# David-Wobrock/image-processing-graph-laplacian

Hardware: AMD Instinct MI355X
Metric: filtered Mpixels/sec @ 4K img, 0.5% samples; PSNR vs PETSc ref (higher is better)
Workload: dtype f32 (f32 storage and accumulation; MFMA operands split into f16 hi+lo pairs = 22 significant bits)

## Files before the change

### image-processing-graph-laplacian_amd/csrc/band_plan.hpp

```cpp
#pragma once
#include <cstdint>
#include <vector>

#if defined(__HIP__) || defined(__CUDACC__)
#define GLF_BAND_HD __host__ __device__
#else
#define GLF_BAND_HD
#endif

namespace glf {

#ifndef BAND_MAXROWS_X
#define BAND_MAXROWS_X 128
#endif
constexpr int BAND_MAXROWS = BAND_MAXROWS_X;
constexpr int BAND_RMAX = 1023;
constexpr unsigned BAND_EMPTY = 0x0000FFFFu;
#ifndef BAND_PB_X
#define BAND_PB_X 2
#endif
#ifndef BAND_NW_X
#define BAND_NW_X 8
#endif
constexpr int BAND_PB = BAND_PB_X, BAND_NW = BAND_NW_X;
// ... 55 lines not shown
    const int i1 = BSEP_KSTEP * ks + BSEP_KSTEP - 1 < count - 1 ? BSEP_KSTEP * ks + BSEP_KSTEP - 1 : count - 1;
    const int first = gcol[band_sep_col(clo, BSEP_KSTEP * ks, nc)], last = gcol[band_sep_col(clo, i1, nc)];
    return first - p1 >= rad || p0 - last >= rad;
}
GLF_BAND_HD inline uint64_t band_sep_tile_entries(const int *gcol, int nc, int width, int tc0, int tile_px, int d, int rad, bool all)
{
    int clo, count;
    band_sep_tile_cols(gcol, nc, width, tc0, tile_px, d, &clo, &count);
    uint64_t n = 0;
    for (int ks = 0; ks < band_sep_ksteps(count); ++ks)
        for (int pt = 0; pt < tile_px / 32; ++pt)
            if (all || !band_sep_block_dead(gcol, nc, clo, count, ks, tc0 + 32 * pt, tc0 + 32 * pt + 31, rad)) n += (uint64_t)BSEP_KSTEP * 32u;
    return n;
}

struct BandGeom {
    int rad = 0;
    double D2 = 0.0;
    std::vector<int> rows, cols, dcmax;
    bool init(const int *grows, int nr, const int *gcols, int nc, double s_loc);
    unsigned band_of(int r) const;
    unsigned window(int cmin, int cmax, int dr, int shift) const;
};

}
```

### image-processing-graph-laplacian_amd/csrc/ctx.hip

```cpp
#include "glf_internal.hpp"

#include <cmath>
#include <cstdlib>

extern "C" {

const char *glf_strerror(int status)
{
    switch (status) {
    case GLF_OK: return "ok";
    case GLF_ERR_INVALID: return "invalid argument";
    case GLF_ERR_NOMEM: return "out of memory";
    case GLF_ERR_HIP: return "HIP runtime error";
    case GLF_ERR_NODEVICE: return "no usable gfx950 device";
    case GLF_ERR_COMM: return "collective callback failed";
    case GLF_ERR_NOCONV: return "eigensolver did not converge";
    case GLF_ERR_IO: return "image I/O error";
    case GLF_ERR_UNSUPPORTED: return "unsupported";
    default: return "unknown status";
    }
}

int glf_ctx_create(glf_ctx **out, int device, void *hip_stream)
{
// ... 33 lines not shown
        }
    for (auto &row : ctx->mv_ev)
        for (auto &e : row)
            if (hipEventCreate(&e) != hipSuccess) {
                delete ctx;
                return GLF_ERR_HIP;
            }
    ctx->comm.rank = 0;
    ctx->comm.size = 1;
    if (const char *mode = std::getenv("GLF_CONTRACTION")) {
        if (std::strcmp(mode, "f32") == 0) ctx->contraction = GLF_CONTRACT_F32_MFMA;
        else if (std::strcmp(mode, "f16s") == 0) ctx->contraction = GLF_CONTRACT_F16_SPLIT;
        else fprintf(stderr, "glf: ignoring GLF_CONTRACTION=%s (expected f32 or f16s)\n", mode);
    }
    if (const char *dbg = std::getenv("GLF_POOL_DEBUG")) ctx->pool_debug = dbg[0] && dbg[0] != '0';
    for (const char *key : {"NYS_PATH", "DEG_PATH", "MV_PATH", "ROWPASS", "ROWPASS_OP", "SWEEP_COLPASS", "COLPASS", "NYS_NO_LUT", "NO_ECR", "NO_NARROW", "NO_FUSED_FILTER", "FILTER_FORM", "BAND_NOSKIP", "PIX_BAND", "EIG_SHARD", "ZMFMA_GROUPS", "GS", "RESIDUAL", "OPERAND_MAXIMA", "VERBOSE"}) {
        char name[32];
        std::snprintf(name, sizeof(name), "GLF_%s", key);
        if (const char *v = std::getenv(name))
            if (glf_ctx_set_tuning(ctx, key, v) != GLF_OK) fprintf(stderr, "glf: ignoring %s=%s\n", name, v);
    }
    *out = ctx;
    return GLF_OK;
}

int glf_ctx_set_tuning(glf_ctx *ctx, const char *key, const char *value)
{
    if (!ctx || !key) return GLF_ERR_INVALID;
    const bool unset = !value || !value[0] || !std::strcmp(value, "auto") || !std::strcmp(value, "default");
    auto is = [&](const char *s) { return value && !std::strcmp(value, s); };
    auto flag = [&]() { return !unset && !is("0"); };
// ... 14 lines not shown
    } else if (!std::strcmp(key, "SWEEP_COLPASS")) {
        if (!unset && !is("segments") && !is("samples")) return GLF_ERR_INVALID;
        t.sweep_samples = is("samples");
    } else if (!std::strcmp(key, "COLPASS")) {
        if (!unset && !is("ws") && !is("v1")) return GLF_ERR_INVALID;
        t.colpass = is("v1") ? 1 : 0;
    } else if (!std::strcmp(key, "NYS_NO_LUT")) t.nys_no_lut = flag();
    else if (!std::strcmp(key, "NO_ECR")) t.no_ecr = flag();
    else if (!std::strcmp(key, "NO_NARROW")) t.no_narrow = flag();
    else if (!std::strcmp(key, "NO_FUSED_FILTER")) t.no_fused_filter = flag();
    else if (!std::strcmp(key, "FILTER_FORM")) {
        if (!unset && !is("sep") && !is("vec") && !is("phi")) return GLF_ERR_INVALID;
        t.filter_form = is("sep") ? 1 : is("vec") ? 2 : is("phi") ? 3 : 0;
    } else if (!std::strcmp(key, "BAND_NOSKIP")) t.band_noskip = flag();
    else if (!std::strcmp(key, "PIX_BAND")) t.pix_band = flag();
    else if (!std::strcmp(key, "ZMFMA_GROUPS")) t.zmfma_groups = flag();
    else if (!std::strcmp(key, "EIG_SHARD")) t.eig_shard = unset ? 0 : is("0") ? 2 : 1;
    else if (!std::strcmp(key, "GS")) {
        if (!unset && !is("seq") && !is("gram")) return GLF_ERR_INVALID;
        t.gs_seq = is("seq");
    } else if (!std::strcmp(key, "RESIDUAL")) {
        if (!unset && !is("sweep") && !is("derived")) return GLF_ERR_INVALID;
        t.residual_sweep = is("sweep");
    } else if (!std::strcmp(key, "OPERAND_MAXIMA")) {
        if (!unset && !is("sweep") && !is("carried")) return GLF_ERR_INVALID;
        t.operand_maxima_sweep = is("sweep");
    } else if (!std::strcmp(key, "VERBOSE")) t.verbose = flag();
    else return GLF_ERR_INVALID;
    return GLF_OK;
}

size_t glf_ctx_cached_bytes(const glf_ctx *ctx)
{
    size_t total = 0;
    if (ctx)
        for (const glf_pool_block &b : ctx->pool)
            if (!b.in_use) total += b.bytes;
    return total;
}

int glf_ctx_debug_violations(const glf_ctx *ctx)
{
    if (!ctx || !ctx->pool_debug) return -1;
    return ctx->pool_violations;
}

int glf_ctx_destroy(glf_ctx *ctx)
{
    if (!ctx) return GLF_OK;
    (void)hipSetDevice(ctx->device);
    (void)hipStreamSynchronize(ctx->stream);
    for (auto &e : ctx->ev)
        if (e) (void)hipEventDestroy(e);
    for (auto &row : ctx->mv_ev)
// ... 331 lines not shown
```

### image-processing-graph-laplacian_amd/csrc/glf_internal.hpp

```cpp
#pragma once

#include <hip/hip_runtime.h>

#include <cmath>
#include <cstdarg>
#include <cstdint>
#include <cstdio>
#include <cstring>
#include <limits>
#include <type_traits>
#include <utility>
#include <vector>

#include "../../include/glf.h"
#include "band_plan.hpp"

struct glf_pool_block {
    void *p;
    size_t bytes;
    bool in_use;
    unsigned last_call = 0;
};

struct glf_tuning {
// ... 2 lines not shown
    int mv_path = 0;
    int rowpass = 0;
    int rowpass_op = 0;
    bool sweep_samples = false;
    int colpass = 0;
    bool nys_no_lut = false;
    bool no_ecr = false;
    bool gs_seq = false;
    bool residual_sweep = false;
    bool zmfma_groups = false;
    int eig_shard = 0;
    bool no_fused_filter = false;
    int filter_form = 0;
    bool band_noskip = false;
    bool pix_band = false;
    bool no_narrow = false;
    bool operand_maxima_sweep = false;
    bool verbose = false;
};

struct glf_native_comm;

struct glf_ctx {
    std::vector<glf_pool_block> pool;
    int device = 0;
    hipStream_t stream = nullptr;
    bool owns_stream = false;
    glf_comm comm{};
    bool has_comm = false;
    glf_native_comm *native = nullptr;
// ... 9 lines not shown
    hipEvent_t cp_ev[2][CP_RING] = {};
    int mv_pending = 0;
    unsigned call_no = 0;
    int mv_count = 0;
    int narrow_sweeps = 0;
    double mv_ms = 0.0, mv_bytes = 0.0;
    float *x0_block = nullptr;
    unsigned x0_p = 0, x0_m = 0, x0_ld = 0;
    unsigned long long x0_seed = 0;
    float *x0_orth = nullptr;
    double *x0_orth_norms = nullptr;
    int x0_orth_form = 0;
    bool x0_orth_fused = false;
    int contraction = GLF_CONTRACT_F16_SPLIT;
    struct { int skipping = 0, lut = 0; } nys_note;
    struct { int path = 0, shape = 0, skipping = 0, chunks = 0, mgroups = 0; double entries = 0.0; } deg_note;
    struct { unsigned kernels = 0, ld = 0, panels = 0, proj_blocks = 0, apply_blocks = 0, strided = 0; } flt_note;
    void *pinned = nullptr;
    void *band_cache[2] = {nullptr, nullptr};
    bool rank_valid = false;
    float rank_s_val = 0.f;
    int rank_R = 0;
    void *rank_ftab = nullptr;
    void *rank_ff = nullptr;
    bool pool_debug = false;
    int pool_violations = 0;
    glf_tuning tune;
};

struct glf_graph {
// ... 660 lines not shown
```

### image-processing-graph-laplacian_amd/csrc/host_util.cpp

```cpp
#include <algorithm>
#include <cmath>
#include <cstdint>
#include <cstdlib>
#include <vector>

#include "../../include/glf.h"
#include "band_plan.hpp"
#include "phi_compact.hpp"
#include "robust_loss.hpp"

namespace {

inline uint64_t rotl64(uint64_t x, int k) { return (x << k) | (x >> (64 - k)); }

struct Xoshiro256ss {
    uint64_t s[4];
    explicit Xoshiro256ss(uint64_t seed)
    {
        for (int i = 0; i < 4; ++i) {
            uint64_t z = (seed += 0x9E3779B97F4A7C15ull);
            z = (z ^ (z >> 30)) * 0xBF58476D1CE4E5B9ull;
            z = (z ^ (z >> 27)) * 0x94D049BB133111EBull;
            s[i] = z ^ (z >> 31);
        }
// ... 201 lines not shown
                    unsigned h = glf::BAND_EMPTY;
                    for (int i = glf::BAND_PAIR * j; i < std::min(nb, glf::BAND_PAIR * (j + 1)); ++i) {
                        const int dr = std::abs(trow0 + w - geom.rows[alo + i]);
                        h = glf::band_win_hull(h, dr < geom.rad ? win[(size_t)dr * nt + t] : glf::BAND_EMPTY);
                    }
                    if (u) u[j] = h;
                    if (glf::band_win_live(h)) steps += (h >> 16) - (h & 0xFFFFu) + 1;
                }
            }
        }
    }
    if (ksteps) *ksteps = steps;
    return GLF_OK;
}

int glf_cluster_update(unsigned k, unsigned dim, const double *scale, const double *sums, const uint64_t *counts, const double *cent_prev,
                       double *cent)
{
    return cluster_update(k, dim, scale, sums, counts, cent_prev, cent);
}

int glf_cluster_update_w(unsigned k, unsigned dim, const double *scale, const double *sums, const double *mass, const double *cent_prev,
                         double *cent)
{
    return cluster_update(k, dim, scale, sums, mass, cent_prev, cent);
}

int glf_cluster_seed(const double *rows, size_t n, unsigned dim, unsigned k, uint64_t seed, double *cent)
{
    return cluster_seed(rows, nullptr, n, dim, k, seed, cent);
// ... 318 lines not shown
```

### image-processing-graph-laplacian_amd/csrc/nystroem_band.inc

```

#ifndef BAND_SETPRIO
#define BAND_SETPRIO 1
#endif
#ifndef BAND_PCOPY
#define BAND_PCOPY 16
#endif
#ifndef BAND_NBUF
#define BAND_NBUF 2
#endif
constexpr unsigned BAND_PSTRIDE = 4u * BAND_PCOPY;
#ifndef BAND_GROWS
#define BAND_GROWS 4
#endif
constexpr int BAND_G = BAND_GROWS;
__host__ __device__ constexpr inline int band_chunk_bytes(int mb) { return mb * 2048 + 256; }
constexpr int BAND_WB = 6;
__host__ __device__ constexpr inline int band_stage_chunks(bool samples)
{
    return samples && 2 * BAND_WB > BAND_NBUF * BAND_G ? 2 * BAND_WB : BAND_NBUF * BAND_G;
}
__host__ __device__ inline unsigned band_lds_bytes(int mb, int nw, int rad, int ksc, bool samples, bool plut = true)
{
    return (plut ? 256u * BAND_PSTRIDE : 0u) + (unsigned)band_stage_chunks(samples) * (unsigned)band_chunk_bytes(mb) + 4u * (unsigned)(rad + 1) + 64u * (unsigned)ksc + 4u * BAND_MAXROWS * (unsigned)(1 + 2 * nw) + 16u;
}
// ... 584 lines not shown
        }
        __syncthreads();
        if (tid < LD) {
            double tot = 0.0;
            for (int w = 0; w < NW; ++w) tot += (double)red[w * LD + tid];
            cpartial[((size_t)blockIdx.y * gridDim.x + blockIdx.x) * LD + tid] = tot;
        }
    }
}

struct BandTables {
    int rad = 0, nr = 0, nc = 0, ksc = 0, width = 0;
    int tile_px = 0, ntiles_px = 0, ntiles_s = 0;
    bool ok = false;
    DevBuf<unsigned> blob;
    size_t o_pexp = 0, o_grid = 0, o_rb_px = 0, o_win_px = 0, o_rb_s = 0, o_win_s = 0, o_dcmax = 0;
    const float *tab() const { return reinterpret_cast<const float *>(blob.p); }
    const float *pexp() const { return reinterpret_cast<const float *>(blob.p + o_pexp); }
    const int *grow() const { return reinterpret_cast<const int *>(blob.p + o_grid); }
    const int *gcol() const { return grow() + nr; }
    const unsigned *rowband_px() const { return blob.p + o_rb_px; }
    const unsigned *win_px() const { return blob.p + o_win_px; }
    const unsigned *rowband_s() const { return blob.p + o_rb_s; }
    const unsigned *win_s() const { return blob.p + o_win_s; }
    const int *dcmax() const { return reinterpret_cast<const int *>(blob.p + o_dcmax); }
    std::vector<unsigned> h_rowband_px;
    double er15_rowsum = 0.0;
    int dc0() const { return geom.dcmax.empty() ? -1 : geom.dcmax[0]; }
    int cols_near_tile(int t) const
    {
        int lo = 0, n = 0;
// ... 39 lines not shown
        nc = g.nc;
        ksc = (int)ceil_div(nc, 16);
        width = width_;
        tile_px = tile_px_;
        hrows = g.rows;
        if (nr > 65535 || ksc > 65535) return GLF_ERR_UNSUPPORTED;
        ntiles_px = want_px ? (int)ceil_div(width, tile_px) : 0;
        ntiles_s = want_s ? (int)ceil_div(nc, 32) : 0;
        const size_t n_tab = 256 + 2 * (size_t)(rad + 1);
        o_pexp = (n_tab + 3) / 4 * 4;
        o_grid = o_pexp + 256 * (size_t)BAND_PCOPY;
        o_rb_px = o_grid + (size_t)nr + nc;
        o_win_px = o_rb_px + (want_px ? (size_t)height : 0);
        o_rb_s = o_win_px + (size_t)rad * ntiles_px;
        o_win_s = o_rb_s + (want_s ? (size_t)nr : 0);
        o_dcmax = o_win_s + (size_t)rad * ntiles_s;
        std::vector<unsigned> h(o_dcmax + (size_t)rad);
        float *htab = reinterpret_cast<float *>(h.data());
        for (int e = 0; e < 256; ++e) htab[e] = (float)std::exp2(-(double)coef.s_val * e * e);
        for (int d = 0; d <= rad; ++d) {
            const double t = (double)coef.s_loc * (double)d * (double)d;
            htab[256 + d] = d < rad ? (float)std::exp2(-t) : 0.f;
            htab[256 + rad + 1 + d] = d < rad ? (float)std::exp2((double)NYS_F16_KSCALE_LOG2 - t) : 0.f;
        }
        for (int i = 0; i < 256 * BAND_PCOPY; ++i) reinterpret_cast<float *>(h.data())[o_pexp + i] = htab[i / BAND_PCOPY];
        for (int a = 0; a < nr; ++a) h[o_grid + a] = (unsigned)g.rows[a];
        for (int b = 0; b < nc; ++b) h[o_grid + nr + b] = (unsigned)g.cols[b];
        const std::vector<int> &dcmax = geom.dcmax;
        for (int dr = 0; dr < rad; ++dr) h[o_dcmax + dr] = (unsigned)dcmax[dr];
        int maxband = 0;
        if (want_px) {
// ... 16 lines not shown
            for (int dr = 0; dr < rad; ++dr) {
                if (dcmax[dr] < 0) continue;
                double n = 0.0;
                for (int b = 0; b < nc; ++b) n += (double)(std::min(width - 1, g.cols[b] + dcmax[dr]) - std::max(0, g.cols[b] - dcmax[dr]) + 1);
                pairs_dr[dr] = n;
            }
        }
        if (want_s) {
            for (int a = 0; a < nr; ++a) {
                const unsigned rb = band_of(g.rows[a]);
                h[o_rb_s + a] = rb;
                maxband = std::max(maxband, (int)(rb >> 16) - (int)(rb & 0xFFFF) + 1);
            }
            for (int dr = 0; dr < rad; ++dr)
                for (int t = 0; t < ntiles_s; ++t) h[o_win_s + (size_t)dr * ntiles_s + t] = geom.window(g.cols[t * 32], g.cols[std::min(nc, (t + 1) * 32) - 1], dr, BAND_BLOCK_SHIFT);
            pairs_dr_s.assign(rad, 0.0);
            for (int dr = 0; dr < rad; ++dr) {
                if (dcmax[dr] < 0) continue;
                double n = 0.0;
                int lo = 0, hi = 0;
                for (int b = 0; b < nc; ++b) {
                    while (lo < nc && g.cols[lo] < g.cols[b] - dcmax[dr]) ++lo;
                    while (hi < nc && g.cols[hi] <= g.cols[b] + dcmax[dr]) ++hi;
                    n += (double)(hi - lo);
                }
                pairs_dr_s[dr] = n;
            }
        }
        if (maxband + 8 > BAND_MAXROWS) return GLF_ERR_UNSUPPORTED;
        GLF_TRY(blob.alloc(ctx, h.size()));
// ... 28 lines not shown
    e->s_loc = coef.s_loc;
    e->s_val = coef.s_val;
    e->width = width;
    e->height = height;
    e->tile_px = tile_px;
    const int rc = e->bt.build(ctx, g, coef, width, height, tile_px, px, !px);
    if (rc != GLF_OK) {
        delete e;
        e = nullptr;
        return rc;
    }
    *out = &e->bt;
    return GLF_OK;
}

#ifndef BAND_NW_S_X
#define BAND_NW_S_X 8
#endif
constexpr int BAND_NW_S = BAND_NW_S_X;

template <int MB, int NS = 0, PixGen G = PixGen::Grey>
static int launch_band_px(glf_ctx *ctx, const BandTables &bt, const uint8_t *d_img, int row0, int nrows, const unsigned char *chunks,
                          const float *inv, float *phi, int phi_ld, const uint8_t *d_mask, const uint32_t *d_idx, unsigned p, int raster,
                          double *cpartial, unsigned long long *evaluated, const BandFilter *flt = nullptr, int64_t pix0 = 0, float nsval = 0.f)
{
    if constexpr (G != PixGen::Grey)
        if (flt || cpartial) return set_error(ctx, GLF_ERR_INVALID, "k_band: the colour and 16-bit formats have no filter epilogue");
    if constexpr (NS == 0 && G == PixGen::Grey)
        if (flt && flt->sig.nsig > 0) {
            if (flt->sig.nsig >= BANDV_MAXNC) return set_error(ctx, GLF_ERR_INVALID, "k_band: %d signal planes", flt->sig.nsig);
// ... 9 lines not shown
    hipLaunchKernelGGL(kern, grid, dim3(BAND_NW * 64), lds, ctx->stream, d_img, bt.width, row0, bt.grow(), bt.gcol(), bt.nr, bt.nc,
                       bt.ksc, bt.tab(), bt.pexp(), bt.rad, bt.rowband_px(), bt.win_px(), bt.ntiles_px, chunks, inv, phi, phi_ld, d_mask, d_idx, p, raster,
                       cpartial, (const float *)nullptr, 0, (const double *)nullptr, 0.f, evaluated, row0 + nrows, flt ? flt->w : (const float *)nullptr,
                       flt ? flt->gain : 0.f, flt ? flt->ysub : 0.f, flt ? flt->out : (uint8_t *)nullptr, flt ? flt->zf : (float *)nullptr,
                       flt ? flt->corr : (float *)nullptr, pix0, flt ? flt->sig : BandSignals{}, ctx->tune.band_noskip ? 1 : 0, nsval);
    GLF_LAUNCH_CHECK(ctx);
    return GLF_OK;
}
inline size_t band_px_wgs(const BandTables &bt, int nrows) { return (size_t)bt.ntiles_px * (size_t)ceil_div(nrows, BAND_NW); }

template <int MB, PixGen G = PixGen::Grey>
static int launch_band_samples(glf_ctx *ctx, const BandTables &bt, const uint8_t *svals, int a0, int nrows, const unsigned char *chunks,
                               const float *inv, float *Y, int y_ld, const float *X, int x_ld, const double *degree, float alpha,
                               unsigned long long *evaluated, float nsval = 0.f)
{
    auto kern = k_band<MB, 1, BAND_NW_S, true, 0, G>;
    const unsigned lds = band_lds_bytes(MB, BAND_NW_S, bt.rad, bt.ksc, true, G == PixGen::Grey);
    GLF_HIP(ctx, hipFuncSetAttribute(reinterpret_cast<const void *>(kern), hipFuncAttributeMaxDynamicSharedMemorySize, (int)lds));
    const dim3 grid((unsigned)bt.ntiles_s, (unsigned)ceil_div(nrows, BAND_NW_S));
    hipLaunchKernelGGL(kern, grid, dim3(BAND_NW_S * 64), lds, ctx->stream, svals, bt.nc, a0, bt.grow(), bt.gcol(), bt.nr, bt.nc, bt.ksc,
                       bt.tab(), bt.pexp(), bt.rad, bt.rowband_s(), bt.win_s(), bt.ntiles_s, chunks, inv, Y, y_ld, (const uint8_t *)nullptr,
                       (const uint32_t *)nullptr, 0u, 1, (double *)nullptr, X, x_ld, degree, alpha, evaluated, a0 + nrows, (const float *)nullptr, 0.f,
                       0.f, (uint8_t *)nullptr, (float *)nullptr, (float *)nullptr, (int64_t)0, BandSignals{}, 0, nsval);
    GLF_LAUNCH_CHECK(ctx);
    return GLF_OK;
}

static int band_prep(glf_ctx *ctx, const float *X, unsigned x_ld, const float *colscale, const void *svals, bool raw, int nr, int nc, int ksc, int mb,
                     unsigned char *chunks, int nch = 1)
{
// ... 120 lines not shown
```

### image-processing-graph-laplacian_amd/glf.py

```python
import collections
import ctypes as C
import functools
import os

import numpy as np
import torch

_HERE = os.path.dirname(os.path.abspath(__file__))
LIB_PATH = os.environ.get("GLF_LIBRARY", os.path.join(_HERE, "libglf.so"))
if not os.path.exists(LIB_PATH):
    raise ImportError(
        "libglf.so not found at %s: build it with `make` (or __graft_entry__.build()); "
        "there is no CPU fallback for the HIP path" % LIB_PATH)
_lib = C.CDLL(LIB_PATH)

OK = 0
ERR_INVALID, ERR_NOMEM, ERR_HIP, ERR_NODEVICE, ERR_COMM, ERR_NOCONV, ERR_IO, ERR_UNSUPPORTED = range(-1, -9, -1)
MAT_DENSE, MAT_DIAG, MAT_KERNEL_B = 0, 1, 2
ROWS_NA, ROWS_SAMPLE_FIRST, ROWS_RASTER = 0, 1, 2
KERNEL_BILATERAL, KERNEL_PHOTOMETRIC, KERNEL_SPATIAL, KERNEL_NLM, KERNEL_BILATERAL_RGB, KERNEL_BILATERAL_U16 = 0, 1, 2, 3, 4, 5
KERNEL_BILATERAL_F32 = 6
KERNEL_BILATERAL_RGBF32 = 7
CONTRACT_F32_MFMA, CONTRACT_F16_SPLIT = 1, 2
FILTER_REFERENCE, FILTER_POC, FILTER_SMOOTH, FILTER_SHARPEN = 0, 1, 2, 3
SAMPLING_UNIFORM, SAMPLING_RANDOM = 0, 1
MULTI_RCCL, MULTI_LOOPBACK = 0, 1
RCCL_ID_BYTES = 128

EXPORTS = [
    "glf_strerror", "glf_ctx_create", "glf_ctx_destroy", "glf_ctx_synchronize", "glf_ctx_last_error",
    "glf_ctx_device_info", "glf_ctx_set_tuning", "glf_ctx_set_comm", "glf_rccl_unique_id", "glf_ctx_set_comm_rccl", "glf_ctx_comm_info", "glf_ctx_comm_counters", "glf_multi_create", "glf_multi_destroy",
    "glf_multi_size", "glf_multi_ctx", "glf_multi_last_error", "glf_multi_image_processing", "glf_shard_rows", "glf_band_plan", "glf_ctx_set_contraction", "glf_malloc", "glf_free", "glf_memcpy_h2d", "glf_memcpy_d2h",
    "glf_memset", "glf_mat_create_dense", "glf_mat_create_diag", "glf_mat_destroy", "glf_mat_get_column", "glf_Sampling",
    "glf_host_free", "glf_random_vectors", "glf_synth_image", "glf_RandomSampling", "glf_ComputeAffinityMatrices",
    "glf_ComputeLaplacianMatrix", "glf_InversePowerIteration", "glf_OrthonormaliseVecs", "glf_NormaliseVecs",
    "glf_InverseDiagMat", "glf_Nystroem", "glf_Permutation", "glf_ComputeResultFromLaplacian", "glf_Sinkhorn", "glf_SinkhornRows", "glf_Orthogonalisation",
    "glf_options_default", "glf_image_processing", "glf_image_processing_capture", "glf_ctx_debug_violations", "glf_ctx_cached_bytes", "glf_image_processing_batch", "glf_EntireComputation", "glf_read_png", "glf_write_png", "glf_read_png_rgb", "glf_write_png_rgb",
    "glf_image_processing_signals", "glf_multi_image_processing_signals",
    "glf_image_processing_rgb", "glf_multi_image_processing_rgb", "glf_image_processing_rgb_capture",
    "glf_image_processing_u16", "glf_multi_image_processing_u16", "glf_image_processing_u16_capture", "glf_read_png16", "glf_write_png16",
    "glf_image_processing_rgb_signals", "glf_image_processing_u16_signals",
    "glf_multi_image_processing_rgb_signals", "glf_multi_image_processing_u16_signals",
    "glf_image_processing_f32", "glf_image_processing_f32_capture", "glf_image_processing_f32_signals",
    "glf_multi_image_processing_f32", "glf_multi_image_processing_f32_signals", "glf_read_pfm", "glf_write_pfm",
    "glf_image_processing_rgbf32", "glf_image_processing_rgbf32_capture", "glf_image_processing_rgbf32_signals",
    "glf_multi_image_processing_rgbf32", "glf_multi_image_processing_rgbf32_signals", "glf_read_pfm_rgb", "glf_write_pfm_rgb",
    "glf_graph_build", "glf_graph_destroy", "glf_graph_get_info", "glf_graph_eigenvalues", "glf_graph_gram", "glf_graph_project",
# ... 595 lines not shown
    def call(first_row, units):
        rc = _lib.glf_band_plan(rows.ctypes.data_as(ip), C.c_int(rows.size), cols.ctypes.data_as(ip), C.c_int(cols.size), C.c_float(h_loc),
                                C.c_int(width), C.c_int(height), C.c_int(row_begin), C.c_int(row_end), C.c_int(pair_stride),
                                C.byref(rad), C.byref(tile_px), C.byref(ntiles), first_row, units, C.byref(ksteps))
        if rc != OK:
            raise GlfError(rc, "band_plan(%d x %d, grid %d x %d)" % (width, height, rows.size, cols.size))
    call(None, None)
    n = max(row_end - row_begin, 0)
    first_row = np.empty(n, dtype=np.int32)
    units = np.empty((n, ntiles.value, pair_stride), dtype=np.uint32)
    call(first_row.ctypes.data_as(ip), units.ctypes.data_as(up))
    return {"rad": rad.value, "tile_px": tile_px.value, "ntiles": ntiles.value, "first_row": first_row, "units": units,
            "ksteps": int(ksteps.value)}


def device_tensor_from_ptr(ptr, count, dtype, device):
    iface = {"shape": (count,), "typestr": "<f8" if dtype == torch.float64 else "<f4",
             "data": (ptr, False), "version": 2, "strides": None}

    class _Holder:
        __cuda_array_interface__ = iface
    return torch.as_tensor(_Holder(), device=device)


def make_comm(rank, size, allreduce, allgather=None):
    def wrap(fn, *extra):
        def cb(user, ptr, count):
            try:
                fn(ptr, count, *extra)
                return 0
# ... 159 lines not shown
        return self

    def __exit__(self, *exc):
        self.close()

    def _check(self, rc, what=""):
        if rc != OK:
            raise GlfError(rc, (what + " " if what else "") + _lib.glf_ctx_last_error(self._ctx).decode())

    def set_contraction(self, mode):
        self._check(_lib.glf_ctx_set_contraction(self._ctx, C.c_int(mode)))

    def synchronize(self):
        self._check(_lib.glf_ctx_synchronize(self._ctx))

    TUNING_KEYS = ("NYS_PATH", "DEG_PATH", "MV_PATH", "ROWPASS", "ROWPASS_OP", "SWEEP_COLPASS", "COLPASS", "NYS_NO_LUT", "NO_ECR", "NO_NARROW", "NO_FUSED_FILTER", "FILTER_FORM", "BAND_NOSKIP", "PIX_BAND", "EIG_SHARD", "ZMFMA_GROUPS", "GS", "RESIDUAL", "OPERAND_MAXIMA", "VERBOSE")

    def set_tuning(self, **kw):
        for k, v in kw.items():
            rc = _lib.glf_ctx_set_tuning(self._ctx, k.encode(), None if v is None else str(v).encode())
            if rc != OK:
                raise GlfError(rc, "set_tuning(%s=%r)" % (k, v))

    def reset_tuning(self):
        self.set_tuning(**{k: None for k in self.TUNING_KEYS})

    def debug_violations(self):
        return int(_lib.glf_ctx_debug_violations(self._ctx))

    def cached_bytes(self):
        return int(_lib.glf_ctx_cached_bytes(self._ctx))

    def device_info(self):
        name = C.create_string_buffer(256)
        cus, mem = C.c_int(), C.c_size_t()
        self._check(_lib.glf_ctx_device_info(self._ctx, name, C.c_size_t(256), C.byref(cus), C.byref(mem)))
        return dict(name=name.value.decode(), num_cus=cus.value, total_mem=mem.value)

    def set_comm_rccl(self, rank, size, unique_id, force=False):
        buf = C.create_string_buffer(bytes(unique_id), RCCL_ID_BYTES)
# ... 1118 lines not shown
```

### include/glf.h

```cpp
#ifndef GLF_H
#define GLF_H

#include <stddef.h>
#include <stdint.h>

#ifdef __cplusplus
extern "C" {
#endif

#define GLF_VERSION 100

enum {
    GLF_OK = 0,
    GLF_ERR_INVALID = -1,
    GLF_ERR_NOMEM = -2,
    GLF_ERR_HIP = -3,
    GLF_ERR_NODEVICE = -4,
    GLF_ERR_COMM = -5,
    GLF_ERR_NOCONV = -6,
    GLF_ERR_IO = -7,
    GLF_ERR_UNSUPPORTED = -8
};
const char *glf_strerror(int status);

// ... 27 lines not shown

typedef struct glf_multi glf_multi;
enum { GLF_MULTI_RCCL = 0, GLF_MULTI_LOOPBACK = 1 };
int glf_multi_create(glf_multi **w, int n, const int *devices, int backend);
int glf_multi_destroy(glf_multi *w);
int glf_multi_size(const glf_multi *w);
glf_ctx *glf_multi_ctx(glf_multi *w, int rank);
const char *glf_multi_last_error(const glf_multi *w);

enum { GLF_CONTRACT_F32_MFMA = 1, GLF_CONTRACT_F16_SPLIT = 2 };
int glf_ctx_set_contraction(glf_ctx *ctx, int mode);
int glf_shard_rows(int height, int rank, int size, int *row0, int *row1);
enum { GLF_BAND_WG_ROWS = 8 };
int glf_band_plan(const int *rows, int nr, const int *cols, int nc, float h_loc, int width, int height, int row_begin, int row_end,
                  int pair_stride, int *rad, int *tile_px, int *ntiles, int *first_row, unsigned *units, uint64_t *ksteps);

int glf_malloc(glf_ctx *ctx, void **dptr, size_t bytes);
int glf_free(glf_ctx *ctx, void *dptr);
int glf_memcpy_h2d(glf_ctx *ctx, void *dst, const void *src, size_t bytes);
int glf_memcpy_d2h(glf_ctx *ctx, void *dst, const void *src, size_t bytes);
int glf_memset(glf_ctx *ctx, void *dst, int value, size_t bytes);

enum { GLF_MAT_DENSE = 0, GLF_MAT_DIAG = 1, GLF_MAT_KERNEL_B = 2 };
enum { GLF_ROWS_NA = 0, GLF_ROWS_SAMPLE_FIRST = 1, GLF_ROWS_RASTER = 2 };
enum { GLF_KERNEL_BILATERAL = 0, GLF_KERNEL_PHOTOMETRIC = 1, GLF_KERNEL_SPATIAL = 2, GLF_KERNEL_NLM = 3, GLF_KERNEL_BILATERAL_RGB = 4,
       GLF_KERNEL_BILATERAL_U16 = 5, GLF_KERNEL_BILATERAL_F32 = 6, GLF_KERNEL_BILATERAL_RGBF32 = 7 };

typedef struct glf_mat {
    int32_t kind;
    int32_t row_order;
// ... 457 lines not shown
```

Measured before the change: 2822.

## Add 2D patch-tiled band sweep kernel for grey-guide Nystroem sample block

Adds a new k_band_sweep kernel where each wave owns a 4x8 patch of target samples (one MFMA tile) instead of a row strip, with per-wave band windows and a workgroup hull that stage source chunks into shared memory through a double-buffered DMA loop. Tighter per-patch windows are meant to skip more dead k-steps and let waves share staged source chunks. It becomes the default for grey guides whenever the window fits six positions and the LDS budget allows; otherwise it falls back to the row form. The cost is more host planning, a larger table blob, and per-pair synchronisation in the kernel.

Result: slower. 2671 (-5.4%).

```diff
diff --git a/image-processing-graph-laplacian_amd/csrc/band_plan.hpp b/image-processing-graph-laplacian_amd/csrc/band_plan.hpp
--- a/image-processing-graph-laplacian_amd/csrc/band_plan.hpp
+++ b/image-processing-graph-laplacian_amd/csrc/band_plan.hpp
@@ -93,6 +93,44 @@
     return n;
 }
 
+#ifndef BAND_SW_NW_X
+#define BAND_SW_NW_X 4
+#endif
+#ifndef BAND_SW_WC_X
+#define BAND_SW_WC_X 2
+#endif
+constexpr int BAND_SW_TR = 4, BAND_SW_TC = 8, BAND_SW_NW = BAND_SW_NW_X, BAND_SW_WC = BAND_SW_WC_X, BAND_SW_WR = BAND_SW_NW / BAND_SW_WC;
+constexpr int BAND_SW_ROWS = BAND_SW_TR * BAND_SW_WR, BAND_SW_COLS = BAND_SW_TC * BAND_SW_WC;
+constexpr int BAND_SW_POS = 6;
+static_assert(BAND_SW_TR * BAND_SW_TC == 32 && BAND_SW_WR * BAND_SW_WC == BAND_SW_NW, "a patch is one MFMA tile of targets");
+GLF_BAND_HD inline unsigned band_sweep_unit(const unsigned *winp, int ntp, int pt, const int *grow, int rad, int t0, int t1, int b0, int b1)
+{
+    unsigned u = BAND_EMPTY;
+    for (int t = t0; t < t1; ++t)
+        for (int b = b0; b < b1; ++b) {
+            const int d = grow[t] - grow[b], dr = d < 0 ? -d : d;
+            if (dr < rad) u = band_win_hull(u, winp[(size_t)dr * ntp + pt]);
+        }
+    return u;
+}
+GLF_BAND_HD inline bool band_sweep_fits(int wave_pos, int maxband) { return wave_pos >= 1 && wave_pos <= BAND_SW_POS && maxband + BAND_SW_ROWS <= BAND_MAXROWS; }
+GLF_BAND_HD inline int band_win_width(unsigned u) { return band_win_live(u) ? (int)(u >> 16) - (int)(u & 0xFFFFu) + 1 : 0; }
+
+GLF_BAND_HD inline void band_sweep_extents(const unsigned *winp, int rad, int ntp, int *wave_pos, int *slots)
+{
+    *wave_pos = *slots = 0;
+    for (int t0 = 0; t0 < ntp; t0 += BAND_SW_WC) {
+        unsigned g = BAND_EMPTY;
+        for (int t = t0; t < ntp && t < t0 + BAND_SW_WC; ++t) {
+            unsigned u = BAND_EMPTY;
+            for (int dr = 0; dr < rad; ++dr) u = band_win_hull(u, winp[(size_t)dr * ntp + t]);
+            if (band_win_width(u) > *wave_pos) *wave_pos = band_win_width(u);
+            g = band_win_hull(g, u);
+        }
+        if (band_win_width(g) > *slots) *slots = band_win_width(g);
+    }
+}
+
 struct BandGeom {
     int rad = 0;
     double D2 = 0.0;
diff --git a/image-processing-graph-laplacian_amd/csrc/ctx.hip b/image-processing-graph-laplacian_amd/csrc/ctx.hip
--- a/image-processing-graph-laplacian_amd/csrc/ctx.hip
+++ b/image-processing-graph-laplacian_amd/csrc/ctx.hip
@@ -71,7 +71,7 @@
         else fprintf(stderr, "glf: ignoring GLF_CONTRACTION=%s (expected f32 or f16s)\n", mode);
     }
     if (const char *dbg = std::getenv("GLF_POOL_DEBUG")) ctx->pool_debug = dbg[0] && dbg[0] != '0';
-    for (const char *key : {"NYS_PATH", "DEG_PATH", "MV_PATH", "ROWPASS", "ROWPASS_OP", "SWEEP_COLPASS", "COLPASS", "NYS_NO_LUT", "NO_ECR", "NO_NARROW", "NO_FUSED_FILTER", "FILTER_FORM", "BAND_NOSKIP", "PIX_BAND", "EIG_SHARD", "ZMFMA_GROUPS", "GS", "RESIDUAL", "OPERAND_MAXIMA", "VERBOSE"}) {
+    for (const char *key : {"NYS_PATH", "DEG_PATH", "MV_PATH", "ROWPASS", "ROWPASS_OP", "SWEEP_COLPASS", "COLPASS", "NYS_NO_LUT", "NO_ECR", "NO_NARROW", "NO_FUSED_FILTER", "FILTER_FORM", "BAND_NOSKIP", "PIX_BAND", "SWEEP_TILE", "EIG_SHARD", "ZMFMA_GROUPS", "GS", "RESIDUAL", "OPERAND_MAXIMA", "VERBOSE"}) {
         char name[32];
         std::snprintf(name, sizeof(name), "GLF_%s", key);
         if (const char *v = std::getenv(name))
@@ -116,6 +116,10 @@
         t.filter_form = is("sep") ? 1 : is("vec") ? 2 : is("phi") ? 3 : 0;
     } else if (!std::strcmp(key, "BAND_NOSKIP")) t.band_noskip = flag();
     else if (!std::strcmp(key, "PIX_BAND")) t.pix_band = flag();
+    else if (!std::strcmp(key, "SWEEP_TILE")) {
+        if (!unset && !is("rows") && !is("patch")) return GLF_ERR_INVALID;
+        t.sweep_tile = is("rows") ? 1 : is("patch") ? 2 : 0;
+    }
     else if (!std::strcmp(key, "ZMFMA_GROUPS")) t.zmfma_groups = flag();
     else if (!std::strcmp(key, "EIG_SHARD")) t.eig_shard = unset ? 0 : is("0") ? 2 : 1;
     else if (!std::strcmp(key, "GS")) {
@@ -140,6 +144,8 @@
             if (!b.in_use) total += b.bytes;
     return total;
 }
+
+int glf_ctx_sweep_form(const glf_ctx *ctx) { return ctx ? ctx->sweep_form : GLF_ERR_INVALID; }
 
 int glf_ctx_debug_violations(const glf_ctx *ctx)
 {
diff --git a/image-processing-graph-laplacian_amd/csrc/glf_internal.hpp b/image-processing-graph-laplacian_amd/csrc/glf_internal.hpp
--- a/image-processing-graph-laplacian_amd/csrc/glf_internal.hpp
+++ b/image-processing-graph-laplacian_amd/csrc/glf_internal.hpp
@@ -40,6 +40,7 @@
     int filter_form = 0;
     bool band_noskip = false;
     bool pix_band = false;
+    int sweep_tile = 0;
     bool no_narrow = false;
     bool operand_maxima_sweep = false;
     bool verbose = false;
@@ -79,6 +80,7 @@
     bool x0_orth_fused = false;
     int contraction = GLF_CONTRACT_F16_SPLIT;
     struct { int skipping = 0, lut = 0; } nys_note;
+    int sweep_form = 0;
     struct { int path = 0, shape = 0, skipping = 0, chunks = 0, mgroups = 0; double entries = 0.0; } deg_note;
     struct { unsigned kernels = 0, ld = 0, panels = 0, proj_blocks = 0, apply_blocks = 0, strided = 0; } flt_note;
     void *pinned = nullptr;
diff --git a/image-processing-graph-laplacian_amd/csrc/host_util.cpp b/image-processing-graph-laplacian_amd/csrc/host_util.cpp
--- a/image-processing-graph-laplacian_amd/csrc/host_util.cpp
+++ b/image-processing-graph-laplacian_amd/csrc/host_util.cpp
@@ -239,6 +239,61 @@
     return GLF_OK;
 }
 
+int glf_band_sweep_plan(const int *rows, int nr, const int *cols, int nc, float h_loc, int row_begin, int row_end, int pair_stride, int *rad,
+                        int *patch_rows, int *patch_cols, int *wg_rows, int *npatch_cols, int *form, int *first_row, unsigned *units,
+                        uint64_t *ksteps, uint64_t *wave_ksteps_max)
+{
+    if (!rows || !cols || nr <= 0 || nc <= 0 || row_begin < 0 || row_end > nr || row_begin > row_end || !(h_loc > 0.f)) return GLF_ERR_INVALID;
+    const float s_loc = (float)(1.4426950408889634 / ((double)h_loc * (double)h_loc));
+    glf::BandGeom geom;
+    if (!geom.init(rows, nr, cols, nc, (double)s_loc)) return GLF_ERR_UNSUPPORTED;
+    constexpr int TR = glf::BAND_SW_TR, TC = glf::BAND_SW_TC, WGR = glf::BAND_SW_ROWS;
+    const int ntp = (nc + TC - 1) / TC;
+    if (rad) *rad = geom.rad;
+    if (patch_rows) *patch_rows = TR;
+    if (patch_cols) *patch_cols = TC;
+    if (wg_rows) *wg_rows = WGR;
+    if (npatch_cols) *npatch_cols = ntp;
+    std::vector<unsigned> winp((size_t)geom.rad * ntp), rowband((size_t)nr);
+    for (int dr = 0; dr < geom.rad; ++dr)
+        for (int t = 0; t < ntp; ++t) winp[(size_t)dr * ntp + t] = geom.window(cols[t * TC], cols[std::min(nc, (t + 1) * TC) - 1], dr, glf::BAND_HALF_SHIFT);
+    int wave_pos = 0, slots = 0, maxband = 0;
+    glf::band_sweep_extents(winp.data(), geom.rad, ntp, &wave_pos, &slots);
+    for (int a = 0; a < nr; ++a) {
+        rowband[a] = geom.band_of(rows[a]);
+        maxband = std::max(maxband, (int)(rowband[a] >> 16) - (int)(rowband[a] & 0xFFFFu) + 1);
+    }
+    const bool patch = glf::band_sweep_fits(wave_pos, maxband);
+    if (form) *form = patch ? 2 : 1;
+    uint64_t steps = 0, wmax = 0;
+    for (int trow0 = row_begin; trow0 < row_end; trow0 += WGR) {
+        const int ntr = std::min(WGR, row_end - trow0);
+        int alo, ahi;
+        glf::band_rows_hull(rowband.data(), trow0, ntr, &alo, &ahi);
+        const int nb = std::min(glf::BAND_MAXROWS, std::max(0, ahi - alo + 1)), npairs = (nb + 1) / 2;
+        if (units && npairs > pair_stride) return GLF_ERR_INVALID;
+        for (int t0 = trow0; t0 < trow0 + ntr; t0 += TR) {
+            const int t1 = std::min(t0 + TR, row_end), pr = (t0 - row_begin) / TR;
+            if (first_row) first_row[pr] = nb > 0 ? alo : -1;
+            for (int pt = 0; pt < ntp; ++pt) {
+                unsigned *u = units ? units + ((size_t)pr * ntp + pt) * (size_t)pair_stride : nullptr;
+                for (int j = 0; u && j < pair_stride; ++j) u[j] = glf::BAND_EMPTY;
+                uint64_t w = 0;
+                for (int j = 0; j < npairs; ++j) {
+                    const unsigned h = glf::band_sweep_unit(winp.data(), ntp, pt, rows, geom.rad, t0, t1, alo + 2 * j, alo + std::min(2 * j + 2, nb));
+                    if (u) u[j] = h;
+                    w += (uint64_t)glf::band_win_width(h);
+                }
+                steps += w;
+                wmax = std::max(wmax, w);
+            }
+        }
+    }
+    if (ksteps) *ksteps = steps;
+    if (wave_ksteps_max) *wave_ksteps_max = wmax;
+    return GLF_OK;
+}
+
 int glf_cluster_update(unsigned k, unsigned dim, const double *scale, const double *sums, const uint64_t *counts, const double *cent_prev,
                        double *cent)
 {
diff --git a/image-processing-graph-laplacian_amd/csrc/nystroem_band.inc b/image-processing-graph-laplacian_amd/csrc/nystroem_band.inc
--- a/image-processing-graph-laplacian_amd/csrc/nystroem_band.inc
+++ b/image-processing-graph-laplacian_amd/csrc/nystroem_band.inc
@@ -622,7 +622,9 @@
     int tile_px = 0, ntiles_px = 0, ntiles_s = 0;
     bool ok = false;
     DevBuf<unsigned> blob;
-    size_t o_pexp = 0, o_grid = 0, o_rb_px = 0, o_win_px = 0, o_rb_s = 0, o_win_s = 0, o_dcmax = 0;
+    size_t o_pexp = 0, o_grid = 0, o_rb_px = 0, o_win_px = 0, o_rb_s = 0, o_win_s = 0, o_win_p = 0, o_dcmax = 0;
+    int ntiles_p = 0, sw_wave_pos = 0, sw_slots = 0, maxband_s = 0;
+    const unsigned *win_p() const { return blob.p + o_win_p; }
     const float *tab() const { return reinterpret_cast<const float *>(blob.p); }
     const float *pexp() const { return reinterpret_cast<const float *>(blob.p + o_pexp); }
     const int *grow() const { return reinterpret_cast<const int *>(blob.p + o_grid); }
@@ -692,7 +694,9 @@
         o_win_px = o_rb_px + (want_px ? (size_t)height : 0);
         o_rb_s = o_win_px + (size_t)rad * ntiles_px;
         o_win_s = o_rb_s + (want_s ? (size_t)nr : 0);
-        o_dcmax = o_win_s + (size_t)rad * ntiles_s;
+        ntiles_p = want_s ? (int)ceil_div(nc, BAND_SW_TC) : 0;
+        o_win_p = o_win_s + (size_t)rad * ntiles_s;
+        o_dcmax = o_win_p + (size_t)rad * ntiles_p;
         std::vector<unsigned> h(o_dcmax + (size_t)rad);
         float *htab = reinterpret_cast<float *>(h.data());
         for (int e = 0; e < 256; ++e) htab[e] = (float)std::exp2(-(double)coef.s_val * e * e);
@@ -739,6 +743,11 @@
             }
             for (int dr = 0; dr < rad; ++dr)
                 for (int t = 0; t < ntiles_s; ++t) h[o_win_s + (size_t)dr * ntiles_s + t] = geom.window(g.cols[t * 32], g.cols[std::min(nc, (t + 1) * 32) - 1], dr, BAND_BLOCK_SHIFT);
+            for (int dr = 0; dr < rad; ++dr)
+                for (int t = 0; t < ntiles_p; ++t)
+                    h[o_win_p + (size_t)dr * ntiles_p + t] = geom.window(g.cols[t * BAND_SW_TC], g.cols[std::min(nc, (t + 1) * BAND_SW_TC) - 1], dr, BAND_HALF_SHIFT);
+            band_sweep_extents(h.data() + o_win_p, rad, ntiles_p, &sw_wave_pos, &sw_slots);
+            maxband_s = maxband;
             pairs_dr_s.assign(rad, 0.0);
             for (int dr = 0; dr < rad; ++dr) {
                 if (dcmax[dr] < 0) continue;
@@ -797,6 +806,8 @@
     return GLF_OK;
 }
 
+#include "nystroem_band_sweep.inc"
+
 #ifndef BAND_NW_S_X
 #define BAND_NW_S_X 8
 #endif
@@ -836,6 +847,17 @@
                                const float *inv, float *Y, int y_ld, const float *X, int x_ld, const double *degree, float alpha,
                                unsigned long long *evaluated, float nsval = 0.f)
 {
+    if constexpr (G != PixGen::Grey)
+        if (ctx->tune.sweep_tile == 2) return set_error(ctx, GLF_ERR_UNSUPPORTED, "SWEEP_TILE=patch: the patch form exists for grey guides only");
+    if constexpr (G == PixGen::Grey) {
+        if (ctx->tune.sweep_tile == 2 && !band_sweep_applies(bt, MB))
+            return set_error(ctx, GLF_ERR_UNSUPPORTED, "SWEEP_TILE=patch: the window of this graph exceeds the patch form's %d positions", BAND_SW_POS);
+        if (ctx->tune.sweep_tile != 1 && band_sweep_applies(bt, MB)) {
+            ctx->sweep_form = 2;
+            return launch_band_sweep<MB>(ctx, bt, svals, a0, nrows, chunks, inv, Y, y_ld, X, x_ld, degree, alpha, evaluated);
+        }
+    }
+    ctx->sweep_form = 1;
     auto kern = k_band<MB, 1, BAND_NW_S, true, 0, G>;
     const unsigned lds = band_lds_bytes(MB, BAND_NW_S, bt.rad, bt.ksc, true, G == PixGen::Grey);
     GLF_HIP(ctx, hipFuncSetAttribute(reinterpret_cast<const void *>(kern), hipFuncAttributeMaxDynamicSharedMemorySize, (int)lds));
diff --git a/image-processing-graph-laplacian_amd/csrc/nystroem_band_sweep.inc b/image-processing-graph-laplacian_amd/csrc/nystroem_band_sweep.inc
--- /dev/null
+++ b/image-processing-graph-laplacian_amd/csrc/nystroem_band_sweep.inc
@@ -0,0 +1,230 @@
+
+#ifndef BAND_SW_NBUF_X
+#define BAND_SW_NBUF_X(mb) ((mb) == 1 ? 2 : 1)
+#endif
+__host__ __device__ constexpr inline int band_sweep_nbuf(int mb) { return BAND_SW_NBUF_X(mb); }
+#ifndef BAND_SW_PCOPY
+#define BAND_SW_PCOPY 4
+#endif
+constexpr unsigned BAND_SW_PBYTES = 256u * 4u * BAND_SW_PCOPY;
+constexpr int BAND_SW_PSHIFT = BAND_PCOPY == 16 * BAND_SW_PCOPY ? 4 : BAND_PCOPY == 8 * BAND_SW_PCOPY ? 3 : BAND_PCOPY == 4 * BAND_SW_PCOPY ? 2 : BAND_PCOPY == 2 * BAND_SW_PCOPY ? 1 : 0;
+static_assert(BAND_PCOPY == (BAND_SW_PCOPY << BAND_SW_PSHIFT), "the sweep's table stride is k_band's shifted down");
+__host__ __device__ inline unsigned band_sweep_lds_bytes(int mb, int nw, int rad, int ksc, int slots)
+{
+    return BAND_SW_PBYTES + (unsigned)band_sweep_nbuf(mb) * (unsigned)slots * (unsigned)band_chunk_bytes(mb) + 8u * (unsigned)(rad + 1) + 64u * (unsigned)ksc +
+           4u * BAND_MAXROWS + 2u * BAND_MAXROWS * (unsigned)(1 + nw) + 8u * (unsigned)nw + 16u;
+}
+
+template <int MB, int NW>
+__global__ __launch_bounds__(NW * 64) void k_band_sweep(const uint8_t *__restrict__ tval, int row_begin, int row_end, const int *__restrict__ grow,
+                                                         const int *__restrict__ gcol, int nr, int nc, int ksc, const float *__restrict__ btab,
+                                                         int rad, const unsigned *__restrict__ rowband,
+                                                         const unsigned *__restrict__ winp, int ntp, int slots, const unsigned char *__restrict__ chunks,
+                                                         const float *__restrict__ inv, float *__restrict__ out, int out_ld, const float *__restrict__ X,
+                                                         int x_ld, const double *__restrict__ degree, float alpha, unsigned long long *__restrict__ evaluated)
+{
+    constexpr int WC = BAND_SW_WC, WR = NW / WC, TR = BAND_SW_TR, TC = BAND_SW_TC, POS = BAND_SW_POS;
+    constexpr int CHB = band_chunk_bytes(MB), NPIECE = MB * 2 + 1, MAXP = BAND_MAXROWS / 2;
+    constexpr int FAR = 1 << 28, NBUF = band_sweep_nbuf(MB);
+    static_assert(NW % WC == 0, "the patches of a workgroup form a rectangle");
+    extern __shared__ __attribute__((aligned(16))) unsigned char bdyn[];
+    float *plut = reinterpret_cast<float *>(bdyn);
+    unsigned char *stage = bdyn + BAND_SW_PBYTES;
+    float *elut = reinterpret_cast<float *>(stage + NBUF * slots * CHB);
+    float *erlut = elut + (rad + 1);
+    int *gcs = reinterpret_cast<int *>(erlut + (rad + 1));
+    int *brow = gcs + 16 * ksc;
+    unsigned *gwin = reinterpret_cast<unsigned *>(brow + BAND_MAXROWS);
+    unsigned *wwin = gwin + MAXP;
+    int *misc = reinterpret_cast<int *>(wwin + NW * MAXP);
+    const int tid = threadIdx.x, lane = tid & 63, wave = __builtin_amdgcn_readfirstlane(tid >> 6), half = lane >> 5, l31 = lane & 31;
+    const int bx = (int)blockIdx.x, by = (int)blockIdx.y;
+    const int trow0 = row_begin + by * (TR * WR);
+    const int ntr = min(TR * WR, row_end - trow0);
+    const int pt = bx * WC + wave % WC;
+    const int wt0 = trow0 + (wave / WC) * TR, wt1 = min(wt0 + TR, row_end);
+    const bool wvalid = pt < ntp && wt0 < wt1;
+    int alo, ahi;
+    band_rows_hull(rowband, trow0, ntr, &alo, &ahi);
+    alo = __builtin_amdgcn_readfirstlane(alo);
+    const int nb = __builtin_amdgcn_readfirstlane(min(BAND_MAXROWS, max(0, ahi - alo + 1))), npairs = (nb + 1) / 2;
+
+    for (int i = tid; i < 256 * BAND_SW_PCOPY; i += NW * 64) plut[i] = btab[i / BAND_SW_PCOPY];
+    for (int i = tid; i <= rad; i += NW * 64) {
+        elut[i] = btab[256 + i];
+        erlut[i] = btab[256 + rad + 1 + i];
+    }
+    for (int i = tid; i < 16 * ksc; i += NW * 64) gcs[i] = i < nc ? gcol[i] : -FAR;
+    for (int i = tid; i < BAND_MAXROWS; i += NW * 64) brow[i] = i < nb ? grow[alo + i] : -FAR;
+    for (int j = tid; j < npairs; j += NW * 64) {
+        unsigned g = BAND_EMPTY;
+        for (int w = 0; w < NW; ++w) {
+            const int t0 = trow0 + (w / WC) * TR, t1 = min(t0 + TR, row_end), ptw = bx * WC + w % WC;
+            const unsigned u = ptw < ntp && t0 < t1 ? band_sweep_unit(winp, ntp, ptw, grow, rad, t0, t1, alo + 2 * j, alo + min(2 * j + 2, nb)) : BAND_EMPTY;
+            wwin[w * MAXP + j] = u;
+            g = band_win_hull(g, u);
+        }
+        gwin[j] = g;
+    }
+    __syncthreads();
+    if (tid < NW) {
+        unsigned u = BAND_EMPTY;
+        for (int j = 0; j < npairs; ++j) u = band_win_hull(u, wwin[tid * MAXP + j]);
+        misc[2 * tid] = (int)(u & 0xFFFFu);
+        misc[2 * tid + 1] = band_win_live(u) ? (int)(u >> 16) : -1;
+    }
+    __syncthreads();
+    const int Wlo = __builtin_amdgcn_readfirstlane(misc[2 * wave]), Whi = __builtin_amdgcn_readfirstlane(misc[2 * wave + 1]);
+
+    const int ta = wt0 + l31 / TC, tb = pt * TC + l31 % TC;
+    const bool tvalid = wvalid && ta < wt1 && tb < nc;
+    const int tac = min(ta, nr - 1), tbc = min(tb, nc - 1);
+    const int Rt = tvalid ? grow[tac] : FAR, tcx = gcol[tbc];
+    const unsigned pv128 = (BAND_PSTRIDE >> BAND_SW_PSHIFT) * (unsigned)tval[(size_t)tac * nc + tbc];
+    const unsigned pbase = lds_offset_of(plut) + 4u * (unsigned)(lane % BAND_SW_PCOPY);
+    f32x16 acc[MB];
+#pragma unroll
+    for (int j = 0; j < MB; ++j)
+#pragma unroll
+        for (int q = 0; q < 16; ++q) acc[j][q] = 0.f;
+    f32x2 ecs[POS][4];
+#pragma unroll
+    for (int bq = 0; bq < POS; ++bq)
+#pragma unroll
+        for (int e = 0; e < 8; ++e) {
+            const int cb = Wlo + bq <= Whi ? gcs[8 * (Wlo + bq) + e] : -FAR;
+            ecs[bq][e >> 1][e & 1] = elut[min(abs(tcx - cb), rad)];
+        }
+
+    const unsigned dma_off_row = 16u * (unsigned)l31, dma_off = dma_off_row + (half ? (unsigned)ksc * CHB : 0u);
+    const unsigned dma_toff_row = 16u * (unsigned)(lane & 1), dma_toff = dma_toff_row + ((lane >> 1) & 1 ? (unsigned)ksc * CHB : 0u);
+    auto live = [&](int j) -> bool { return band_win_live(gwin[j]); };
+    auto next_pair = [&](int j) -> int {
+        do ++j;
+        while (j < npairs && !live(j));
+        return j;
+    };
+    auto issue = [&](int j, int bf) {
+        const unsigned u = (unsigned)__builtin_amdgcn_readfirstlane((int)gwin[j]);
+        const int lo = (int)(u & 0xFFFFu), n = min(band_win_width(u), slots), i = 2 * j;
+        const bool both = i + 1 < nb;
+        for (int q = wave; q < n * NPIECE; q += NW) {
+            const int slot = q / NPIECE, k = q % NPIECE, hb = lo + slot;
+            const unsigned dst = (unsigned)__builtin_amdgcn_readfirstlane((int)lds_offset_of(stage + (size_t)(bf * slots + slot) * CHB + k * 1024));
+            const unsigned char *ch = chunks + ((size_t)(alo + i) * ksc + (hb >> 1)) * CHB + k * 1024;
+            if (k < NPIECE - 1) lds_dma_16B_base(ch + 512 * (hb & 1), both ? dma_off : dma_off_row, dst);
+            else if (lane < 4) lds_dma_16B_base(ch + 32 * (hb & 1), both ? dma_toff : dma_toff_row, dst);
+        }
+    };
+    auto kstep = [&](const unsigned char *sl, float era, const f32x2 (&ec)[4]) __attribute__((always_inline)) {
+        const uint4 s0 = *reinterpret_cast<const uint4 *>(sl + MB * 2048 + 32 * half);
+        const uint4 s1 = *reinterpret_cast<const uint4 *>(sl + MB * 2048 + 32 * half + 16);
+        const unsigned sv128[8] = {s0.x, s0.y, s0.z, s0.w, s1.x, s1.y, s1.z, s1.w};
+        float pp[8];
+#pragma unroll
+        for (int e = 0; e < 8; ++e) pp[e] = lds_f32(sad_u32(pv128, sv128[e] >> BAND_SW_PSHIFT, pbase));
+        __builtin_amdgcn_sched_barrier(0);
+        f16x8 ah, al;
+#pragma unroll
+        for (int e = 0; e < 8; e += 2) {
+            f32x2 y;
+            y[0] = (era * ec[e >> 1][0]) * pp[e];
+            y[1] = (era * ec[e >> 1][1]) * pp[e + 1];
+            const f16x2 h2 = __builtin_convertvector(y, f16x2);
+            f32x2 res;
+            res[0] = y[0] - (float)h2[0];
+            res[1] = y[1] - (float)h2[1];
+            const f16x2 l2 = __builtin_convertvector(res, f16x2);
+            ah[e] = h2[0];
+            ah[e + 1] = h2[1];
+            al[e] = l2[0];
+            al[e + 1] = l2[1];
+        }
+        if (BAND_SETPRIO) __builtin_amdgcn_s_setprio(1);
+#pragma unroll
+        for (int j = 0; j < MB; ++j) {
+            const f16x8 bh = *reinterpret_cast<const f16x8 *>(sl + (j * 2 + 0) * 1024 + lane * 16);
+            const f16x8 bl = *reinterpret_cast<const f16x8 *>(sl + (j * 2 + 1) * 1024 + lane * 16);
+            acc[j] = __builtin_amdgcn_mfma_f32_32x32x16_f16(ah, bh, acc[j], 0, 0, 0);
+            acc[j] = __builtin_amdgcn_mfma_f32_32x32x16_f16(ah, bl, acc[j], 0, 0, 0);
+            acc[j] = __builtin_amdgcn_mfma_f32_32x32x16_f16(al, bh, acc[j], 0, 0, 0);
+        }
+        if (BAND_SETPRIO) __builtin_amdgcn_s_setprio(0);
+    };
+
+    unsigned long long nsteps = 0;
+    int j = npairs > 0 && live(0) ? 0 : next_pair(0), bf = 0;
+    if (npairs <= 0) j = 0;
+    if (j < npairs) issue(j, 0);
+    lds_dma_drain();
+    __syncthreads();
+    while (j < npairs) {
+        const int jn = next_pair(j);
+        if (NBUF > 1 && jn < npairs) issue(jn, bf ^ 1);
+        if (wvalid) {
+            const unsigned ug = (unsigned)__builtin_amdgcn_readfirstlane((int)gwin[j]);
+            const unsigned uw = (unsigned)__builtin_amdgcn_readfirstlane((int)wwin[wave * MAXP + j]);
+            if (band_win_live(uw)) {
+                const int glo = (int)(ug & 0xFFFFu), ie = 2 * j + half;
+                const int rb = ie < nb ? brow[ie] : -FAR;
+                const float era = erlut[min(abs(Rt - rb), rad)];
+                const unsigned char *sb = stage + (size_t)bf * slots * CHB;
+#pragma unroll
+                for (int bq = 0; bq < POS; ++bq) {
+                    const int hb = Wlo + bq;
+                    if (band_win_has(uw, hb) && hb - glo < slots) {
+                        kstep(sb + (size_t)(hb - glo) * CHB, era, ecs[bq]);
+                        ++nsteps;
+                    }
+                }
+            }
+        }
+        if (NBUF == 1) {
+            __syncthreads();
+            if (jn < npairs) issue(jn, 0);
+        }
+        lds_dma_drain();
+        __syncthreads();
+        j = jn;
+        bf = NBUF > 1 ? bf ^ 1 : 0;
+    }
+    if (evaluated && lane == 0 && nsteps) atomicAdd(evaluated, nsteps * (unsigned long long)(16 * 32));
+
+    if (!wvalid) return;
+    float iv[MB];
+#pragma unroll
+    for (int jj = 0; jj < MB; ++jj) iv[jj] = inv[32 * jj + l31];
+#pragma unroll
+    for (int q = 0; q < 16; ++q) {
+        const int t = (q & 3) + 8 * (q >> 2) + 4 * half;
+        const int a = wt0 + t / TC, b = pt * TC + t % TC;
+        if (a >= wt1 || b >= nc) continue;
+        const size_t s = (size_t)a * nc + b;
+        const float dg = (float)degree[s];
+#pragma unroll
+        for (int jj = 0; jj < MB; ++jj)
+            out[s * out_ld + 32 * jj + l31] = alpha * fmaf(dg, X[s * x_ld + 32 * jj + l31], -(acc[jj][q] * iv[jj]));
+    }
+}
+
+static bool band_sweep_applies(const BandTables &bt, int mb)
+{
+    return band_sweep_fits(bt.sw_wave_pos, bt.maxband_s) && bt.sw_slots >= 1 &&
+           band_sweep_lds_bytes(mb, BAND_SW_NW, bt.rad, bt.ksc, bt.sw_slots) <= 160u * 1024u;
+}
+
+template <int MB>
+static int launch_band_sweep(glf_ctx *ctx, const BandTables &bt, const uint8_t *svals, int a0, int nrows, const unsigned char *chunks,
+                             const float *inv, float *Y, int y_ld, const float *X, int x_ld, const double *degree, float alpha,
+                             unsigned long long *evaluated)
+{
+    auto kern = k_band_sweep<MB, BAND_SW_NW>;
+    const unsigned lds = band_sweep_lds_bytes(MB, BAND_SW_NW, bt.rad, bt.ksc, bt.sw_slots);
+    GLF_HIP(ctx, hipFuncSetAttribute(reinterpret_cast<const void *>(kern), hipFuncAttributeMaxDynamicSharedMemorySize, (int)lds));
+    const dim3 grid((unsigned)ceil_div(bt.ntiles_p, BAND_SW_WC), (unsigned)ceil_div(nrows, BAND_SW_ROWS));
+    hipLaunchKernelGGL(kern, grid, dim3(BAND_SW_NW * 64), lds, ctx->stream, svals, a0, a0 + nrows, bt.grow(), bt.gcol(), bt.nr, bt.nc, bt.ksc,
+                       bt.tab(), bt.rad, bt.rowband_s(), bt.win_p(), bt.ntiles_p, bt.sw_slots, chunks, inv, Y, y_ld, X, x_ld, degree,
+                       alpha, evaluated);
+    GLF_LAUNCH_CHECK(ctx);
+    return GLF_OK;
+}
diff --git a/image-processing-graph-laplacian_amd/glf.py b/image-processing-graph-laplacian_amd/glf.py
--- a/image-processing-graph-laplacian_amd/glf.py
+++ b/image-processing-graph-laplacian_amd/glf.py
@@ -30,7 +30,7 @@
 EXPORTS = [
     "glf_strerror", "glf_ctx_create", "glf_ctx_destroy", "glf_ctx_synchronize", "glf_ctx_last_error",
     "glf_ctx_device_info", "glf_ctx_set_tuning", "glf_ctx_set_comm", "glf_rccl_unique_id", "glf_ctx_set_comm_rccl", "glf_ctx_comm_info", "glf_ctx_comm_counters", "glf_multi_create", "glf_multi_destroy",
-    "glf_multi_size", "glf_multi_ctx", "glf_multi_last_error", "glf_multi_image_processing", "glf_shard_rows", "glf_band_plan", "glf_ctx_set_contraction", "glf_malloc", "glf_free", "glf_memcpy_h2d", "glf_memcpy_d2h",
+    "glf_multi_size", "glf_multi_ctx", "glf_multi_last_error", "glf_multi_image_processing", "glf_shard_rows", "glf_band_plan", "glf_band_sweep_plan", "glf_ctx_sweep_form", "glf_ctx_set_contraction", "glf_malloc", "glf_free", "glf_memcpy_h2d", "glf_memcpy_d2h",
     "glf_memset", "glf_mat_create_dense", "glf_mat_create_diag", "glf_mat_destroy", "glf_mat_get_column", "glf_Sampling",
     "glf_host_free", "glf_random_vectors", "glf_synth_image", "glf_RandomSampling", "glf_ComputeAffinityMatrices",
     "glf_ComputeLaplacianMatrix", "glf_InversePowerIteration", "glf_OrthonormaliseVecs", "glf_NormaliseVecs",
@@ -656,6 +656,30 @@
             "ksteps": int(ksteps.value)}
 
 
+def band_sweep_plan(rows, cols, h_loc=40.0, row_begin=0, row_end=None, pair_stride=64):
+    rows = np.ascontiguousarray(rows, dtype=np.int32)
+    cols = np.ascontiguousarray(cols, dtype=np.int32)
+    row_end = rows.size if row_end is None else row_end
+    rad, tr, tc, wgr, npc, form = (C.c_int() for _ in range(6))
+    ksteps, wmax = C.c_uint64(), C.c_uint64()
+    ip, up = C.POINTER(C.c_int), C.POINTER(C.c_uint)
+
+    def call(first_row, units):
+        rc = _lib.glf_band_sweep_plan(rows.ctypes.data_as(ip), C.c_int(rows.size), cols.ctypes.data_as(ip), C.c_int(cols.size), C.c_float(h_loc),
+                                      C.c_int(row_begin), C.c_int(row_end), C.c_int(pair_stride), C.byref(rad), C.byref(tr), C.byref(tc),
+                                      C.byref(wgr), C.byref(npc), C.byref(form), first_row, units, C.byref(ksteps), C.byref(wmax))
+        if rc != OK:
+            raise GlfError(rc, "band_sweep_plan(grid %d x %d)" % (rows.size, cols.size))
+    call(None, None)
+    n = -(-max(row_end - row_begin, 0) // tr.value)
+    first_row = np.empty(n, dtype=np.int32)
+    units = np.empty((n, npc.value, pair_stride), dtype=np.uint32)
+    call(first_row.ctypes.data_as(ip), units.ctypes.data_as(up))
+    return {"rad": rad.value, "patch_rows": tr.value, "patch_cols": tc.value, "wg_rows": wgr.value, "npatch_cols": npc.value,
+            "form": "patch" if form.value == 2 else "rows", "first_row": first_row, "units": units, "ksteps": int(ksteps.value),
+            "wave_ksteps_max": int(wmax.value)}
+
+
 def device_tensor_from_ptr(ptr, count, dtype, device):
     iface = {"shape": (count,), "typestr": "<f8" if dtype == torch.float64 else "<f4",
              "data": (ptr, False), "version": 2, "strides": None}
@@ -845,7 +869,7 @@
     def synchronize(self):
         self._check(_lib.glf_ctx_synchronize(self._ctx))
 
-    TUNING_KEYS = ("NYS_PATH", "DEG_PATH", "MV_PATH", "ROWPASS", "ROWPASS_OP", "SWEEP_COLPASS", "COLPASS", "NYS_NO_LUT", "NO_ECR", "NO_NARROW", "NO_FUSED_FILTER", "FILTER_FORM", "BAND_NOSKIP", "PIX_BAND", "EIG_SHARD", "ZMFMA_GROUPS", "GS", "RESIDUAL", "OPERAND_MAXIMA", "VERBOSE")
+    TUNING_KEYS = ("NYS_PATH", "DEG_PATH", "MV_PATH", "ROWPASS", "ROWPASS_OP", "SWEEP_COLPASS", "COLPASS", "NYS_NO_LUT", "NO_ECR", "NO_NARROW", "NO_FUSED_FILTER", "FILTER_FORM", "BAND_NOSKIP", "PIX_BAND", "SWEEP_TILE", "EIG_SHARD", "ZMFMA_GROUPS", "GS", "RESIDUAL", "OPERAND_MAXIMA", "VERBOSE")
 
     def set_tuning(self, **kw):
         for k, v in kw.items():
@@ -855,6 +879,9 @@
 
     def reset_tuning(self):
         self.set_tuning(**{k: None for k in self.TUNING_KEYS})
+
+    def sweep_form(self):
+        return {1: "rows", 2: "patch"}.get(int(_lib.glf_ctx_sweep_form(self._ctx)))
 
     def debug_violations(self):
         return int(_lib.glf_ctx_debug_violations(self._ctx))
diff --git a/include/glf.h b/include/glf.h
--- a/include/glf.h
+++ b/include/glf.h
@@ -65,6 +65,11 @@
 enum { GLF_BAND_WG_ROWS = 8 };
 int glf_band_plan(const int *rows, int nr, const int *cols, int nc, float h_loc, int width, int height, int row_begin, int row_end,
                   int pair_stride, int *rad, int *tile_px, int *ntiles, int *first_row, unsigned *units, uint64_t *ksteps);
+
+int glf_band_sweep_plan(const int *rows, int nr, const int *cols, int nc, float h_loc, int row_begin, int row_end, int pair_stride, int *rad,
+                        int *patch_rows, int *patch_cols, int *wg_rows, int *npatch_cols, int *form, int *first_row, unsigned *units,
+                        uint64_t *ksteps, uint64_t *wave_ksteps_max);
+int glf_ctx_sweep_form(const glf_ctx *ctx);
 
 int glf_malloc(glf_ctx *ctx, void **dptr, size_t bytes);
 int glf_free(glf_ctx *ctx, void *dptr);
```
